# linyicheng1/keypoint_bench

Measured on AMD Instinct MI355X. Metric: image-pairs/sec (extract+NMS+BF-match, 640x480, top_k=1000), higher is better.
Workload: dtype f32

## Files before the change

### include/kpb.h

```cpp
#ifndef KPB_H
#define KPB_H

#include <stddef.h>
#include <stdint.h>

#ifdef __cplusplus
extern "C" {
#endif

#define KPB_VERSION 1

#define KPB_OK 0
#define KPB_E_INVALID (-1)
#define KPB_E_HIP (-2)
#define KPB_E_NOMEM (-3)
#define KPB_E_NEGATIVE (-4)
#define KPB_E_NOT_CONVERGED (-5)
#define KPB_E_WEIGHTS (-6)
#define KPB_E_UNSUPPORTED (-7)

#define KPB_MAX_NMS_DIST 16
#define KPB_MAX_TOPK 8192

typedef struct kpb_ctx kpb_ctx;
// ... 1 lines not shown

typedef struct kpb_detect_params {
    int32_t nms_dist;
    float threshold;
    int32_t border_dist;
    int32_t top_k;
    float min_score;
} kpb_detect_params;

typedef struct kpb_match_params {
    double max_distance;
    int32_t cross_check;
} kpb_match_params;

int kpb_version(void);
const char* kpb_last_error(const kpb_ctx* ctx);

int kpb_ctx_create(int device, void* stream, kpb_ctx** out);
int kpb_ctx_set_stream(kpb_ctx* ctx, void* stream);
void kpb_ctx_destroy(kpb_ctx* ctx);
int kpb_sync(kpb_ctx* ctx);

#define KPB_OPT_COVIS_STORE_BYTES 1
int kpb_ctx_set_option(kpb_ctx* ctx, int option, int64_t value);

int kpb_prof_enable(kpb_ctx* ctx, int on);
int kpb_prof_report(kpb_ctx* ctx, char* buf, size_t cap);

int kpb_fast_nms(kpb_ctx* ctx, const float* score_dev, int batch, int H, int W, int nms_dist,
                 float* out_map_dev);

int kpb_detect(kpb_ctx* ctx, const float* score_dev, int batch, int H, int W,
               const kpb_detect_params* params, float* out_kps_dev, int32_t* out_idx_dev,
               int32_t* out_n_dev, int sync);
int kpb_detect_check(kpb_ctx* ctx);
int kpb_detect_counts(kpb_ctx* ctx, int32_t* out_n_host, int batch);

int kpb_sample(kpb_ctx* ctx, const float* desc_dev, int batch, int C, int Hd, int Wd, int64_t sb,
               int64_t sc, int64_t sh, int64_t sw, const float* pts_dev, int pts_cols, int max_n,
               const int32_t* n_dev, float* out_dev);

int kpb_match(kpb_ctx* ctx, const float* d0_dev, const float* d1_dev, int batch, int C, int max_n,
              int max_m, const int32_t* n_dev, const int32_t* m_dev, const kpb_match_params* params,
              int32_t* out_pairs_dev, double* out_dist_dev, int32_t* out_k_dev);

int kpb_match_counts(kpb_ctx* ctx, int32_t* out_k_host, int batch);
// ... 92 lines not shown
```

### keypoint_bench_amd/_lib.py

```python
import ctypes
import os

_HERE = os.path.dirname(os.path.abspath(__file__))
SO_PATH = os.environ.get("KPB_LIB_PATH") or os.path.join(_HERE, "libkpb.so")

c_int, c_float, c_double, c_void_p, c_int64, c_size_t = (ctypes.c_int, ctypes.c_float, ctypes.c_double,
                                                       ctypes.c_void_p, ctypes.c_int64, ctypes.c_size_t)


class DetectParams(ctypes.Structure):
    _fields_ = [("nms_dist", ctypes.c_int32), ("threshold", c_float), ("border_dist", ctypes.c_int32),
                ("top_k", ctypes.c_int32), ("min_score", c_float)]


class LgParams(ctypes.Structure):
    _fields_ = [("depth_confidence", c_float), ("width_confidence", c_float), ("filter_threshold", c_float),
                ("prune_min_kpts", ctypes.c_int32)]


class LkParams(ctypes.Structure):
    _fields_ = [("distance", ctypes.c_float), ("win_size", ctypes.c_int32), ("levels", ctypes.c_int32), ("iterations", ctypes.c_int32)]


class RansacParams(ctypes.Structure):
# ... 106 lines not shown
    @classmethod
    def get(cls, device):
        import torch
        idx = device.index if isinstance(device, torch.device) else int(device)
        if idx is None:
            idx = torch.cuda.current_device()
        if idx not in cls._instances:
            cls._instances[idx] = cls(idx)
        inst = cls._instances[idx]
        stream = torch.cuda.current_stream(idx).cuda_stream
        if stream != inst.stream:
            inst.check(inst.lib.kpb_ctx_set_stream(inst.handle, c_void_p(stream)))
            inst.stream = stream
        return inst

    def check(self, rc):
        if rc != 0:
            raise KpbError(rc, self.lib.kpb_last_error(self.handle).decode())

    def sync(self):
        self.check(self.lib.kpb_sync(self.handle))

    OPT_COVIS_STORE_BYTES = 1

    def set_option(self, option: int, value: int):
        self.check(self.lib.kpb_ctx_set_option(self.handle, int(option), int(value)))

    def prof_enable(self, on: bool):
        self.check(self.lib.kpb_prof_enable(self.handle, 1 if on else 0))

    def prof_report(self):
        buf = ctypes.create_string_buffer(1 << 16)
        self.check(self.lib.kpb_prof_report(self.handle, buf, len(buf)))
        out = {}
        for line in buf.value.decode().splitlines():
            name, calls, ms = line.split()
            out[name] = (int(calls), float(ms))
        return out


def ptr(t):
    return c_void_p(t.data_ptr()) if t is not None else c_void_p(0)
```

### keypoint_bench_amd/csrc/alike.hip

```cpp
#include "conv_mfma.h"

namespace {

typedef _Float16 h8v __attribute__((ext_vector_type(8)));
typedef _Float16 h2v __attribute__((ext_vector_type(2)));
typedef float f32x4v __attribute__((ext_vector_type(4)));

__device__ __forceinline__ float relu(float v);

__device__ __forceinline__ void split4(const float4 v, uint2& hi, uint2& lo) { cm_split4(v, hi, lo); }

__device__ __forceinline__ void amax_commit(float lane_max, float* slots, int slot, int lane)
{
    const float m = cm_wave_max(lane_max);
    if (lane == 0) slots[slot] = m;
}

__global__ __launch_bounds__(256) void amax_reduce(const float* slots, int n, unsigned* out)
{
    __shared__ float s[4];
    const int b = blockIdx.x, tid = threadIdx.x;
    float m = 0.0f;
    for (int i = tid; i < n; i += 256) {
        const float v = slots[(size_t)b * n + i];
// ... 752 lines not shown

std::vector<float> pack_h16(const float* w, int CIN, const float* ds_w, float scale)
{
    const int OCT = CIN / 8, NK = 9 * OCT + (ds_w ? 1 : 0), KB = (NK + 3) / 4;
    std::vector<uint16_t> hl((size_t)KB * 2 * 64 * 8, 0);
    for (int kb = 0; kb < KB; ++kb)
        for (int l = 0; l < 64; ++l)
            for (int j = 0; j < 8; ++j) {
                const int n = l & 15, g = l >> 4, kidx = 4 * kb + g;
                float v = 0.0f;
                if (kidx < 9 * OCT) { const int tap = kidx / OCT, o = kidx - tap * OCT; v = w[((size_t)n * CIN + 8 * o + j) * 9 + tap]; }
                else if (ds_w && kidx == 9 * OCT) v = ds_w[n * 8 + j];
                v *= scale;
                _Float16 hi = (_Float16)v;
                const _Float16 lo = (_Float16)(v - (float)hi);
                memcpy(&hl[(((size_t)kb * 2 + 0) * 64 + l) * 8 + j], &hi, 2);
                memcpy(&hl[(((size_t)kb * 2 + 1) * 64 + l) * 8 + j], &lo, 2);
            }
    std::vector<float> out(hl.size() / 2);
    memcpy(out.data(), hl.data(), hl.size() * 2);
    return out;
}

constexpr int ESTRIDE = 68;

template <int CIN>
__device__ __forceinline__ void conv1x1_relu_body(const float* __restrict__ in, float* __restrict__ out, const float* __restrict__ w ,
                                                  const float* __restrict__ wsg , float* __restrict__ smap, size_t npix,
                                                  const float* __restrict__ wproj , float* __restrict__ E ,
                                                  const unsigned bx )
{
    const size_t p = (size_t)bx * 256 + threadIdx.x;
    const bool live = p < npix;
    constexpr bool STAGE_IN = CIN <= 32;
    constexpr int XP = CIN + 4;
    constexpr int WREG = STAGE_IN && 64 * XP > 16 * ESTRIDE ? 64 * XP : 16 * ESTRIDE;
    __shared__ __attribute__((aligned(16))) float wlds[4][WREG];
    float* wreg = wlds[threadIdx.x >> 6];
    float acc[16];
#pragma unroll
    for (int j = 0; j < 16; ++j) acc[j] = 0.0f;
    const float* x = in + (live ? p : 0) * CIN;
    if (STAGE_IN) {
        const int ln = threadIdx.x & 63;
        const size_t pw = (size_t)bx * 256 + (threadIdx.x >> 6) * 64;
        float4 ld[CIN / 4];
#pragma unroll
// ... 821 lines not shown
    for (int o = 0; o < co; ++o)
        for (int c = 0; c < ci; ++c) out[(size_t)c * co + o] = w[(size_t)o * ci + c];
}
float l1_rows(const float* w, int co, int per)
{
    float m = 0.0f;
    for (int o = 0; o < co; ++o) {
        double s = 0.0;
        for (int i = 0; i < per; ++i) s += std::fabs((double)w[(size_t)o * per + i]);
        m = std::max(m, (float)(s * (1.0 + 1e-6)));
    }
    return m;
}
float max_abs(const float* b, int n)
{
    float m = 0.0f;
    for (int i = 0; i < n; ++i) m = std::max(m, std::fabs(b[i]));
    return m;
}

constexpr CmForm CM_C16{.ks = 3, .s = 1, .cc = 16, .ntb = 1, .mt = 2, .wn = 2}, CM_C32{.ks = 3, .s = 1, .cc = 32, .ntb = 1, .mt = 4, .wn = 2},
                 CM_C32_1T{.ks = 3, .s = 1, .cc = 32, .ntb = 1}, CM_C16_LAT{.ks = 3, .s = 1, .cc = 16, .wpre = true},
                 CM_C32_LAT{.ks = 3, .s = 1, .cc = 32, .ntb = 1, .wpre = true}, CM_P4_LAT{.ks = 3, .s = 1, .cc = 32, .pool_in = true, .ntb = 1, .pf = 4, .wpre = true};

template <int CIN, int COUT, int POOL, bool RES, int CDS, int RPOOL, bool DSOUT = false, int TW = 32>
void launch_conv(kpb_ctx* ctx, const char* name, hipStream_t st, const ConvArgs& a, int B)
{
    constexpr int G = COUT / 16, TH = (64 / TW) * (4 / G);
    KPB_LAUNCH(ctx, name, (conv3x3_k<CIN, COUT, POOL, RES, CDS, RPOOL, true, DSOUT, TW>), dim3(cdiv(a.W, TW), cdiv(a.H, TH), B), dim3(256), 0, st, a);
}

__global__ __launch_bounds__(256) void maxpool4_nhwc(const float* __restrict__ in, float* __restrict__ out, int Ho, int Wo, int C)
{
    const int C4 = C / 4;
    const size_t i = (size_t)blockIdx.x * 256 + threadIdx.x, b = blockIdx.y;
    if (i >= (size_t)Ho * Wo * C4) return;
    const int c = (int)(i % C4) * 4;
    const size_t pix = i / C4;
    const int y = (int)(pix / Wo), x = (int)(pix - (size_t)y * Wo);
    const float* s = in + ((b * 4 * Ho + 4 * y) * (size_t)(4 * Wo) + 4 * x) * C + c;
    float4 m = *reinterpret_cast<const float4*>(s);
#pragma unroll
    for (int py = 0; py < 4; ++py)
#pragma unroll
        for (int px = 0; px < 4; ++px) {
            if (py == 0 && px == 0) continue;
            const float4 v = *reinterpret_cast<const float4*>(s + ((size_t)py * 4 * Wo + px) * C);
            m.x = fmaxf(m.x, v.x); m.y = fmaxf(m.y, v.y); m.z = fmaxf(m.z, v.z); m.w = fmaxf(m.w, v.w);
        }
    *reinterpret_cast<float4*>(out + ((b * Ho + y) * (size_t)Wo + x) * C + c) = m;
}

int AlikeNet::forward(const float* img_dev, int batch, int H_, int W_, float* score_out_dev, float* desc_out_dev)
{
    if ((H_ % 32) || (W_ % 32))
        return kpb_fail(ctx, KPB_E_INVALID, "kpb_net_forward: ALIKE needs H and W multiples of 32 (got %dx%d)", H_, W_);
    const int H = H_, W = W_;
    const size_t P = (size_t)H * W, B = batch;
    const bool h16 = conv_mfma_use_h16();
    const bool dense = desc_out_dev != nullptr;
    const int nw1 = cdiv(W, B1_TW) * cdiv(H, B1H_TH) * 4, nw2 = cdiv(W / 2, 32) * cdiv(H / 2, 8) * 4;
    const size_t n_2 = B * (P / 4) * 16, n_3 = B * (P / 64) * 32, n_4 = B * (P / 1024) * 64;
    float *p1, *t2, *x2, *t3, *x3, *t4, *x4, *r3, *r4, *t3r3, *t4r4, *p2, *p3, *S2, *S3, *S4, *E3, *E4, *wmax_x1, *wmax_a2;
    unsigned *amax_x1, *amax_a2;
    if (int rc = kpb_carve(ctx, act, [&](Arena& a) {
            auto f32 = [&](size_t n) { return h16 ? nullptr : a.take(n); };
            auto f16 = [&](size_t n) { return h16 ? a.take(n) : nullptr; };
            x1 = a.take(B * P * 8);
            p1 = a.take(B * (P / 4) * 8);
            t2 = f32(n_2); x2 = f32(n_2); a2 = a.take(n_2);
            t3 = f32(n_3); x3 = a.take(n_3); a3 = a.take(B * (P / 64) * 16);
            t4 = f32(n_4); x4 = a.take(n_4); a4 = a.take(B * (P / 1024) * 16);
            r3 = f32(n_3); r4 = f32(n_4);
            t3r3 = f16(2 * n_3);
            t4r4 = f16(2 * n_4);
            p2 = f16(n_3 / 2);
            p3 = h16 && batch >= 16 ? a.take(n_4 / 2) : nullptr;
            S2 = a.take(B * (P / 4)); S3 = a.take(B * (P / 64)); S4 = a.take(B * (P / 1024));
            E3 = dense ? a.take(B * (P / 64) * ESTRIDE) : nullptr;
            E4 = dense ? a.take(B * (P / 1024) * ESTRIDE) : nullptr;
            amax_x1 = h16 ? a.take<unsigned>(B) : nullptr;
            amax_a2 = h16 ? a.take<unsigned>(B) : nullptr;
            wmax_x1 = f16(B * nw1);
            wmax_a2 = f16(B * nw2);
        }))
        return rc;
    this->B = batch; this->H = H; this->W = W;
    hipStream_t st = ctx->stream;

    Block1Args b1{img_dev, x1, p1, k1.w1, k1.b1, k1.w2, k1.b2, H, W};
    ConvArgs c;
    if (h16) {
        Block1HArgs hb{b1, k1.w1pk, k1.w2pk, k1.inv_ws1, k1.inv_ws2, k1.l1_c1, k1.bmax_c1, wmax_x1, 0};
        KPB_LAUNCH(ctx, "alike_block1", alike_block1_h, dim3(cdiv(W, B1_TW), cdiv(H, B1H_TH), batch), dim3(256), 0, st, hb);
        KPB_LAUNCH(ctx, "amax_reduce", amax_reduce, dim3(batch), dim3(256), 0, st, wmax_x1, nw1, amax_x1);
        Block2Args b2{p1, x2, a2, S2, p2, k2.w1pk, k2.w2pk, k2.wapk, k2.b1, k2.bsum, kh.wsc + 16, H / 2, W / 2,
                      k2.inv_ws1, k2.inv_ws2, k2.inv_wsa, k2.l1_c1, k2.bmax_c1, k2.l1_c2, k2.l1_ds, k2.bmax_sum, amax_x1, wmax_a2, 1};
        KPB_LAUNCH(ctx, "alike_block2", alike_block2, dim3(cdiv(W / 2, 32), cdiv(H / 2, 8), batch), dim3(256), 0, st, b2);
        KPB_LAUNCH(ctx, "amax_reduce", amax_reduce, dim3(batch), dim3(256), 0, st, wmax_a2, nw2, amax_a2);
        auto block_h = [&](const Res& r, const float* in, float* tr, float* xo, int cin, int cout, int Hi, int Wi, bool prepooled) {
            ConvM m{.in = in, .out = tr, .wp = r.w1h, .bias = r.b1h, .Hi = prepooled ? Hi / 4 : Hi, .Wi = prepooled ? Wi / 4 : Wi,
                    .H = Hi / 4, .W = Wi / 4, .CIN = cin, .COUT = 2 * cout, .NCH = 1, .relu = 2, .nblk = cout / 32, .istride = cin, .ostride = 2 * cout,
                    .unscale = r.un1, .relu_nt = cout / 32};
            auto launch = [&](const char* prof, const CmForm& f, const ConvM& cm) {
                return launch_conv_mfma_h<CM_C16, CM_C32, CM_C32_1T, CM_C16_LAT, CM_C32_LAT, CM_P4_LAT>(ctx, prof, f, cm, batch); };
            if (batch < 16 && !prepooled) m.nblk = 2 * cout / 32;
            const CmForm f1 = !prepooled ? CM_P4_LAT : batch < 16 ? CM_C16_LAT : cin == 32 ? CM_C32 : CM_C16;
            if (int rc = launch(r.prof1.c_str(), f1, m)) return rc;
            const ConvM c2{.in = tr, .out = xo, .wp = r.w2p, .bias = r.b2p, .res = tr + cout, .Hi = Hi / 4, .Wi = Wi / 4,
                           .H = Hi / 4, .W = Wi / 4, .CIN = cout, .COUT = cout, .NCH = cout / 32, .nblk = batch < 16 ? cout / 32 : 1, .istride = 2 * cout,
                           .ostride = cout, .unscale = r.un2, .rstride = 2 * cout};
            return launch(r.prof2.c_str(), batch < 16 ? CM_C32_LAT : cout == 32 ? CM_C32_1T : CM_C32, c2);
        };
        if (int rc = block_h(blk[3], p2, t3r3, x3, 16, 32, H / 2, W / 2, true)) return rc;
        if (batch >= 16) {
            KPB_LAUNCH(ctx, "maxpool4_x3", maxpool4_nhwc, dim3((unsigned)(((size_t)(H / 32) * (W / 32) * 8 + 255) / 256), batch), dim3(256), 0, st, x3, p3, H / 32, W / 32, 32);
            if (int rc = block_h(blk[4], p3, t4r4, x4, 32, 64, H / 8, W / 8, true)) return rc;
        } else if (int rc = block_h(blk[4], x3, t4r4, x4, 32, 64, H / 8, W / 8, false))
            return rc;
    } else {
        auto conv2 = [&](const Res& r, const float* in, float* out, const float* res, int h, int w, int c) {
            const ConvM m{.in = in, .out = out, .wp = r.w2p, .bias = r.b2p, .res = res, .Hi = h, .Wi = w, .H = h, .W = w,
                          .CIN = c, .COUT = c, .NCH = c / 32, .nblk = 1, .istride = c, .ostride = c};
            return launch_conv_mfma<CmForm{.ks = 3, .s = 1, .cc = 32, .ntb = 1}, CmForm{.ks = 3, .s = 1, .cc = 32}>(
                ctx, r.prof2.c_str(), CmForm{.ks = 3, .s = 1, .cc = 32, .ntb = c / 32}, m, batch);
        };
        KPB_LAUNCH(ctx, "alike_block1", alike_block1, dim3(cdiv(W, B1_TW), cdiv(H, B1_TH), batch), dim3(256), 0, st, b1);
        c = ConvArgs{p1, t2, blk[2].w1, blk[2].b1, nullptr, nullptr, nullptr, nullptr, H / 2, W / 2};
        launch_conv<8, 16, 1, false, 4, 1>(ctx, "conv3x3_b2c1", st, c, batch);
        c = ConvArgs{t2, x2, blk[2].w2, blk[2].b2, p1, blk[2].dsw, blk[2].dsb, nullptr, H / 2, W / 2};
        launch_conv<16, 16, 1, true, 8, 1>(ctx, "conv3x3_b2c2", st, c, batch);
        c = ConvArgs{x2, t3, blk[3].w1, blk[3].b1, nullptr, blk[3].dsw, blk[3].dsb, r3, H / 8, W / 8};
        launch_conv<16, 32, 4, false, 4, 1, true, 16>(ctx, "conv3x3_b3c1", st, c, batch);
        if (int rc = conv2(blk[3], t3, x3, r3, H / 8, W / 8, 32)) return rc;
        c = ConvArgs{x3, t4, blk[4].w1, blk[4].b1, nullptr, blk[4].dsw, blk[4].dsb, r4, H / 32, W / 32};
        launch_conv<32, 64, 4, false, 4, 1, true, 16>(ctx, "conv3x3_b4c1", st, c, batch);
        if (int rc = conv2(blk[4], t4, x4, r4, H / 32, W / 32, 64)) return rc;
        KPB_LAUNCH(ctx, "conv1x1_agg2", conv1x1_relu<16>, dim3((unsigned)((B * P / 4 + 255) / 256)), dim3(256), 0, st, x2, a2, kh.agg[2], kh.wsc + 16, S2, B * P / 4, nullptr, nullptr);
    }
    if (batch < 16) {
        const AggArgs g3{x3, a3, kh.agg[3], kh.wsc + 32, S3, B * P / 64, kh.whT + 32 * 64, E3};
        const AggArgs g4{x4, a4, kh.agg[4], kh.wsc + 48, S4, B * P / 1024, kh.whT + 48 * 64, E4};
        const unsigned nb3 = (unsigned)((B * P / 64 + 255) / 256), nb4 = (unsigned)((B * P / 1024 + 255) / 256);
        KPB_LAUNCH(ctx, "conv1x1_agg34", conv1x1_relu_34, dim3(nb3 + nb4), dim3(256), 0, st, g3, g4, nb3);
    } else {
        KPB_LAUNCH(ctx, "conv1x1_agg3", conv1x1_relu<32>, dim3((unsigned)((B * P / 64 + 255) / 256)), dim3(256), 0, st, x3, a3, kh.agg[3], kh.wsc + 32, S3, B * P / 64, kh.whT + 32 * 64, E3);
        KPB_LAUNCH(ctx, "conv1x1_agg4", conv1x1_relu<64>, dim3((unsigned)((B * P / 1024 + 255) / 256)), dim3(256), 0, st, x4, a4, kh.agg[4], kh.wsc + 48, S4, B * P / 1024, kh.whT + 48 * 64, E4);
    }
    if (dense) {
        HybArgs hy{x1, a2, E3, E4, kh.agg[1], kh.whT, kh.wsc, score_out_dev, desc_out_dev, H, W, amax_x1, amax_a2, 0.f, 1.f, 1.f, nullptr, 1.f};
        const int work4 = cdiv(H, 4) * cdiv(W / 32, SEG_TILES);
        if (h16) {
            hy.l1_agg1 = kh.l1_agg1; hy.inv_ws_h = kh.inv_ws_h; hy.ws_h = 1.0f / hy.inv_ws_h;
            hy.a1h16 = kh.a1h16; hy.inv_wa = kh.inv_wa;
            if (!hp_ring_rows_ok(H, H / 2, HP_A2R) || !hp_ring_rows_ok(H, H / 8, HP_ER) || !hp_ring_rows_ok(H, H / 32, HP_ER))
                return kpb_fail(ctx, KPB_E_UNSUPPORTED, "alike head: the LDS rings cannot hold the source rows of %d row groups at height %d", HP_LA + 1, H);
            const int bands_ = cdiv(W / 32, HP_TILES), groups_ = H / 4;
            const int hp = std::max(2, std::min(30, (int)(((long long)bands_ * groups_ * batch) / 1536)));
            KPB_LAUNCH(ctx, "alike_head_dense", alike_head_f16p, dim3(cdiv(W / 32, HP_TILES) * cdiv(H / 4, hp), batch), dim3(256), 0, st, hy,
                       kh.wh16, hp);
        } else
            KPB_LAUNCH(ctx, "alike_head_dense", alike_head_hyb, dim3(work4, batch), dim3(256), 0, st, hy);
    } else {
// ... 185 lines not shown
```

### keypoint_bench_amd/csrc/api.hip

```cpp
#include "kpb_common.h"

char g_kpb_err[512] = {0};

extern "C" __attribute__((visibility("default"))) int kpb_version(void) { return KPB_VERSION; }

extern "C" __attribute__((visibility("default"))) const char* kpb_last_error(const kpb_ctx* ctx) { return ctx ? ctx->err : g_kpb_err; }

extern "C" __attribute__((visibility("default"))) int kpb_ctx_create(int device, void* stream, kpb_ctx** out)
{
    if (!out) return kpb_fail(nullptr, KPB_E_INVALID, "kpb_ctx_create: null out pointer");
    *out = nullptr;
    int count = 0;
    if (hipGetDeviceCount(&count) != hipSuccess || count == 0)
        return kpb_fail(nullptr, KPB_E_HIP, "kpb_ctx_create: no HIP device visible (this library has no CPU path)");
    if (device < 0 || device >= count)
        return kpb_fail(nullptr, KPB_E_INVALID, "kpb_ctx_create: device %d out of range (0..%d)", device, count - 1);
    hipDeviceProp_t prop;
    KPB_HIP(nullptr, hipGetDeviceProperties(&prop, device));
    if (strncmp(prop.gcnArchName, "gfx950", 6) != 0)
        return kpb_fail(nullptr, KPB_E_HIP, "kpb_ctx_create: device %d is %s; libkpb.so is built for gfx950 only", device,
                        prop.gcnArchName);
    KPB_HIP(nullptr, hipSetDevice(device));
    kpb_ctx* c = new kpb_ctx();
    c->device = device;
// ... 12 lines not shown
    if (ctx->wait_ev) (void)hipEventDestroy(ctx->wait_ev);
    if (ctx->host_det) (void)hipHostFree(ctx->host_det);
    if (ctx->host_match) (void)hipHostFree(ctx->host_match);
    if (ctx->own_stream) (void)hipStreamDestroy(ctx->stream);
    if (ctx->det_state && ctx->det_state_free) ctx->det_state_free(ctx->det_state);
    for (hipEvent_t e : ctx->prof_pool) (void)hipEventDestroy(e);
    delete ctx;
}

extern "C" __attribute__((visibility("default"))) int kpb_ctx_set_stream(kpb_ctx* ctx, void* stream)
{
    if (!ctx) return kpb_fail(nullptr, KPB_E_INVALID, "kpb_ctx_set_stream: null context");
    KPB_HIP(ctx, hipStreamSynchronize(ctx->stream));
    ctx->stream = static_cast<hipStream_t>(stream);
    return KPB_OK;
}

extern "C" __attribute__((visibility("default"))) int kpb_ctx_set_option(kpb_ctx* ctx, int option, int64_t value)
{
    if (!ctx) return kpb_fail(nullptr, KPB_E_INVALID, "kpb_ctx_set_option: null context");
    if (value < 0) return kpb_fail(ctx, KPB_E_INVALID, "kpb_ctx_set_option: negative value");
    switch (option) {
    case KPB_OPT_COVIS_STORE_BYTES: ctx->covis_store_bytes = (size_t)value; return KPB_OK;
    default: return kpb_fail(ctx, KPB_E_INVALID, "kpb_ctx_set_option: unknown option %d", option);
    }
}

extern "C" __attribute__((visibility("default"))) int kpb_sync(kpb_ctx* ctx)
{
    if (!ctx) return kpb_fail(nullptr, KPB_E_INVALID, "kpb_sync: null context");
    KPB_HIP(ctx, hipStreamSynchronize(ctx->stream));
    return KPB_OK;
}

extern "C" __attribute__((visibility("default"))) int kpb_prof_enable(kpb_ctx* ctx, int on)
{
    if (!ctx) return kpb_fail(nullptr, KPB_E_INVALID, "kpb_prof_enable: null context");
    ctx->prof = on != 0;
    return KPB_OK;
}

extern "C" __attribute__((visibility("default"))) int kpb_prof_report(kpb_ctx* ctx, char* buf, size_t cap)
{
    if (!ctx || !buf || cap == 0) return kpb_fail(ctx, KPB_E_INVALID, "kpb_prof_report: bad argument");
    KPB_HIP(ctx, hipStreamSynchronize(ctx->stream));
    std::vector<std::string> names;
// ... 23 lines not shown
```

### keypoint_bench_amd/csrc/conv_mfma.h

```cpp
#pragma once
#include <type_traits>
#include "net.h"

#include <algorithm>
#include <cmath>
#include <cstring>

namespace {

typedef float f32x16 __attribute__((ext_vector_type(16)));

__device__ __forceinline__ float relu(float v) { return fmaxf(v, 0.0f); }

struct ConvM {
    const float* in = nullptr;
    float* out = nullptr;
    const float* wp = nullptr;
    const float* bias = nullptr;
    const float* xf = nullptr;
    const int* active = nullptr;
    const float* res = nullptr;
    int Hi = 0, Wi = 0, H = 0, W = 0, CIN = 0, COUT = 0, NCH = 0, relu = 0, nblk = 0;
    int istride = 0, ostride = 0, ooff = 0;
    float unscale = 1.0f;
    int relu_nt = 0;
    int rstride = 0;
    const float* xw = nullptr;
    float xun = 1.0f;
    const float* gen_w = nullptr; const float* gen_b = nullptr;
    float xb = 0.0f;
    int xco = 0;
    const int* rowcnt = nullptr;
    const float* aux0 = nullptr;
    const float* aux1 = nullptr;
    float* out1 = nullptr;
    float* out2 = nullptr;
    const unsigned* pre_amax = nullptr; float pre_l1 = 0.0f, pre_bmax = 0.0f;
    const float* up_src = nullptr; int up_c = 0;
    int unfold_w = 0;
    int tap_dil = 0;
};

enum { GE_PLAIN = 0, GE_RESIDUAL = 1, GE_ROTARY = 2, GE_SPLIT2 = 3, GE_L2NORM = 4 };

struct CmForm {
    int ks, s, cc;
    bool pool_in, pool_out;
    bool xf;
    int ntb = 2;
    int mt = 1;
    bool xc = false;
    int pf = 2;
    bool wpre = false;
    bool pre = false;
    int wn = 1;
    bool gen = false;
    bool up = false;
    int dil = 1;
    constexpr bool operator==(const CmForm&) const = default;
    constexpr int tile_h() const { return 8 * mt / wn; }
    constexpr int waves() const { return wpre ? 1 : dil > 1 ? 2  : mt * ntb >= 4 ? ((ks == 5 && cc == 32) || pool_in ? 2 : 3) : (mt * ntb == 2 ? (ks == 3 && cc == 16 ? 3 : 4) : 5); }
};

template <CmForm F>
__global__ __launch_bounds__(256) void conv_mfma(ConvM a)
{
    constexpr int KS = F.ks, S = F.s, CC = F.cc, NTB = F.ntb; constexpr bool POOL_IN = F.pool_in, POOL_OUT = F.pool_out, XF = F.xf;
    constexpr int DIL = F.dil;
    static_assert(F == CmForm{.ks = KS, .s = S, .cc = CC, .pool_in = POOL_IN, .pool_out = POOL_OUT, .xf = XF, .ntb = NTB, .dil = DIL},
                  "conv_mfma: the strict-fp32 kernel has no mt, xc, pf, wpre, pre, wn, gen or up");
    constexpr int KC = CC / 2, PITCH = CC + 4, T = KS * KS, PAD = (KS - 1) * DIL / 2;
    constexpr int IH = 7 * S + (KS - 1) * DIL + 1, IW = 15 * S + (KS - 1) * DIL + 1, Q = CC / 4;
    static_assert(IH * IW * PITCH * 4 <= 65536, "conv_mfma: input tile exceeds the static LDS window");
    constexpr int NLD = (IH * IW * Q + 255) / 256;
    __shared__ __attribute__((aligned(16))) float tile[IH * IW * PITCH];
    const int tid = threadIdx.x, lane = tid & 63, wv = tid >> 6, p = lane & 31, h = lane >> 5;
    const int b = blockIdx.z / a.nblk, nb = blockIdx.z - b * a.nblk, nt0 = nb * NTB;
    const int ty0 = blockIdx.y * 8, tx0 = blockIdx.x * 16;
    const int Hc = POOL_IN ? a.Hi / 2 : a.Hi, Wc = POOL_IN ? a.Wi / 2 : a.Wi;
    const int iy0 = ty0 * S - PAD, ix0 = tx0 * S - PAD;
    if (a.active && !a.active[b]) return;
    const float* in = a.in + (size_t)b * a.Hi * a.Wi * a.istride;
    const int orow = 2 * wv + (p >> 4), ocol = p & 15;
    const size_t ntile_stride = (size_t)T * a.NCH * 2 * 32 * KC;

    f32x16 acc[NTB];
#pragma unroll
    for (int n = 0; n < NTB; ++n)
#pragma unroll
        for (int r = 0; r < 16; ++r) acc[n][r] = 0.0f;
    for (int ch = 0; ch < a.NCH; ++ch) {
        __syncthreads();
        {
// ... 145 lines not shown
        return fmaxf(x, __int_as_float(y));
    };
    v = step(v, std::integral_constant<int, 0xB1>{}, std::integral_constant<int, 0xF>{});
    v = step(v, std::integral_constant<int, 0x4E>{}, std::integral_constant<int, 0xF>{});
    v = step(v, std::integral_constant<int, 0x141>{}, std::integral_constant<int, 0xF>{});
    v = step(v, std::integral_constant<int, 0x140>{}, std::integral_constant<int, 0xF>{});
    v = step(v, std::integral_constant<int, 0x142>{}, std::integral_constant<int, 0xA>{});
    v = step(v, std::integral_constant<int, 0x143>{}, std::integral_constant<int, 0xC>{});
    return __int_as_float(__builtin_amdgcn_readlane(__float_as_int(v), 63));
}

__device__ __forceinline__ void cm_up2_taps(int o, int n, int& i0, int& i1, float& l)
{
    const float f = fmaxf(((float)o + 0.5f) * 0.5f - 0.5f, 0.0f);
    i0 = (int)f;
    i1 = i0 + (i0 < n - 1 ? 1 : 0);
    l = f - (float)i0;
}
__device__ __forceinline__ float4 cm_up2_mix(const float4 p00, const float4 p01, const float4 p10, const float4 p11, float ly, float lx)
{
    const float hy = 1.0f - ly, hx = 1.0f - lx;
    return make_float4(hy * (hx * p00.x + lx * p01.x) + ly * (hx * p10.x + lx * p11.x), hy * (hx * p00.y + lx * p01.y) + ly * (hx * p10.y + lx * p11.y),
                       hy * (hx * p00.z + lx * p01.z) + ly * (hx * p10.z + lx * p11.z), hy * (hx * p00.w + lx * p01.w) + ly * (hx * p10.w + lx * p11.w));
}

template <CmForm F>
__global__ __launch_bounds__(256, F.waves()) void conv_mfma_h(ConvM a)
{
    constexpr int KS = F.ks, S = F.s, CC = F.cc, NTB = F.ntb, MT = F.mt, PF = F.pf, WN = F.wn, DIL = F.dil;
    constexpr bool POOL_IN = F.pool_in, POOL_OUT = F.pool_out, XF = F.xf, XC = F.xc, WPRE = F.wpre, PRE = F.pre, GEN = F.gen, UP = F.up;
    static_assert(DIL == 1 || (DIL >= 2 && S == 1 && !WPRE && !PRE && !UP && !XC && !POOL_IN && MT >= 2 && NTB == 1), "conv_mfma_h: the dilated form exists for plain stride-1 layers (R2D2)");
    static_assert(!UP || (S == 1 && !POOL_IN && !PRE && !WPRE && (((F.tile_h() - 1) * S + KS) % 2 == 0) && ((15 * S + KS) % 2 == 0) && KS / 2 % 2 == 0),
                  "conv_mfma_h<UP>: stride-1 layers whose input tile starts on an even row and column");
    static_assert(WN == 1 || (WN == 2 && MT % 2 == 0 && !WPRE), "conv_mfma_h: waves split the n-tiles two ways at most");
    static_assert(PRE == GEN && (!GEN || KS == 3), "conv_mfma_h: the pre-split tile exists as the generated one (a 3 x 3 one-channel layer computed while staging); r05's DMA-landed form was measured, superseded and removed in r06");
    static_assert(!PRE || (CC == 32 && S == 1 && !POOL_IN && !XF && !XC && !WPRE), "conv_mfma_h: the pre-split input form exists for plain stride-1 32-channel slabs");
    constexpr int KC = CC / 2, NKB = CC / 16, T = KS * KS, PAD = (KS - 1) * DIL / 2, TH = F.tile_h();
    constexpr int TAPU = (KS == 3 && !WPRE && !PRE) ? 9 : 1;
    constexpr bool ROW_AHEAD = TAPU == 1 && !WPRE && !PRE;
    constexpr int IH = (TH - 1) * S + (KS - 1) * DIL + 1, IW = 15 * S + (KS - 1) * DIL + 1, Q = CC / 4;
    constexpr int PITCH = 4 * CC + 16, LO = 2 * CC;
    constexpr int ROWP = (IW * PITCH + 255) / 256 * 256;
    constexpr int NLD = (IH * IW * Q + 255) / 256;
    static_assert(IH * ROWP <= 65536, "conv_mfma_h: input tile exceeds the static LDS window");
    __shared__ __attribute__((aligned(256))) unsigned char tile[IH * ROWP];
    const int tid = threadIdx.x, lane = tid & 63, wv = tid >> 6, p = lane & 31, h = lane >> 5;
// ... 364 lines not shown
#pragma unroll
                    for (int j = 0; j < 4; ++j) {
                        const uint2 w = xwq[4 * q + j];
                        xpart = __builtin_amdgcn_fdot2(__builtin_bit_cast(cm_h2, ll[j]), __builtin_bit_cast(cm_h2, w.x), xpart, false);
                        xpart = __builtin_amdgcn_fdot2(__builtin_bit_cast(cm_h2, hh[j]), __builtin_bit_cast(cm_h2, w.y), xpart, false);
                        xpart = __builtin_amdgcn_fdot2(__builtin_bit_cast(cm_h2, hh[j]), __builtin_bit_cast(cm_h2, w.x), xpart, false);
                    }
                }
            }
        }
        }
        if (XC && nb == 0) xacc = fmaf(xpart, cm_unscale_of(e_cur), xacc);
    }
    if (XC && nb == 0) {
        const int gy = ty0 + (tid >> 4), gx = tx0 + (tid & 15);
        if (gy < a.H && gx < a.W) {
            float o = fmaf(xacc, a.xun, a.xb);
            if (a.relu) o = relu(o);
            a.out[(size_t)b * a.H * a.W * a.ostride + a.ooff + ((size_t)gy * a.W + gx) * a.ostride + a.xco] = o;
        }
    }
    const float unscale = a.unscale * cm_unscale_of(e_cur);

#pragma unroll
    for (int m = 0; m < MT; ++m) {
        const int trow = 2 * (wm * MT + m);
#pragma unroll
        for (int n = 0; n < NTB; ++n) {
            const int co = (nt0 + n) * 32 + p;
            const float bias = biasv[n];
            float v[16];
#pragma unroll
            for (int r = 0; r < 16; ++r) {
                v[r] = fmaf(acc[m][n][r], unscale, bias);
                if (a.relu == 1 || (a.relu == 2 && nt0 + n < a.relu_nt)) v[r] = relu(v[r]);
            }
            if (co >= a.COUT) continue;
            if (!POOL_OUT) {
                float* out = a.out + (size_t)b * a.H * a.W * a.ostride + a.ooff;
                const int rs = a.rstride ? a.rstride : a.COUT;
                const float* res = a.res ? a.res + (size_t)b * a.H * a.W * rs : nullptr;
#pragma unroll
                for (int r = 0; r < 16; ++r) {
                    const int i = (r & 3) + 8 * (r >> 2) + 4 * h;
                    const int gy = ty0 + trow + (i >> 4), gx = tx0 + (i & 15);
                    if (gy < a.H && gx < a.W) {
// ... 11 lines not shown
                const int gy = (ty0 + trow) / 2;
#pragma unroll
                for (int cc = 0; cc < 4; ++cc) {
                    const int c = 2 * h + (cc & 1) + 4 * (cc >> 1);
                    const int rA = 2 * (cc & 1) + 4 * (cc >> 1);
                    const int gx = tx0 / 2 + c;
                    if (gy < Ho && gx < Wo)
                        out[((size_t)gy * Wo + gx) * a.ostride + co] = fmaxf(fmaxf(v[rA], v[rA + 1]), fmaxf(v[rA + 8], v[rA + 9]));
                }
            }
        }
    }
}

template <bool H, CmForm... FS>
int cm_launch(kpb_ctx* ctx, const char* tag, const CmForm& f, const ConvM& a, int B)
{
    const bool found = ((f == FS && [&] {
        const dim3 grid(cdiv(a.W, 16), cdiv(a.H, FS.tile_h()), B * a.nblk);
        if constexpr (H) KPB_LAUNCH(ctx, tag, conv_mfma_h<FS>, grid, dim3(256), 0, ctx->stream, a);
        else KPB_LAUNCH(ctx, tag, conv_mfma<FS>, grid, dim3(256), 0, ctx->stream, a);
        return true;
    }()) || ...);
    return found ? KPB_OK : kpb_fail(ctx, KPB_E_INVALID, "%s: no instance for %s: ks=%d s=%d cc=%d pool_in=%d pool_out=%d xf=%d ntb=%d mt=%d xc=%d pf=%d wpre=%d pre=%d wn=%d gen=%d up=%d dil=%d",
        H ? "conv_mfma_h" : "conv_mfma", tag, f.ks, f.s, f.cc, f.pool_in, f.pool_out, f.xf, f.ntb, f.mt, f.xc, f.pf, f.wpre, f.pre, f.wn, f.gen, f.up, f.dil);
}
template <CmForm... FS> int launch_conv_mfma_h(kpb_ctx* ctx, const char* tag, const CmForm& f, const ConvM& a, int B) { return cm_launch<true, FS...>(ctx, tag, f, a, B); }
template <CmForm... FS> int launch_conv_mfma(kpb_ctx* ctx, const char* tag, const CmForm& f, const ConvM& a, int B) { return cm_launch<false, FS...>(ctx, tag, f, a, B); }

template <int NTB, int MT = 2, int EPI = GE_PLAIN, bool UNFOLD = false, int TAPK = 0>
__global__ __launch_bounds__(256, MT == 1 ? (EPI == GE_ROTARY || TAPK ? 3 : 4) : 2) void gemm_h(ConvM a)
{
    constexpr int CC = 32, KC = 16, NKB = 2, Q = CC / 4, PITCH = 4 * CC + 16, LO = 2 * CC, WROWS = 32 * MT, ROWS = 4 * WROWS, WBUF = WROWS * PITCH,
                  NLD = WROWS * Q / 64;
    __shared__ __attribute__((aligned(256))) unsigned char tile[2 * 4 * WBUF];
    const int tid = threadIdx.x, lane = tid & 63, wv = tid >> 6, p = lane & 31, h = lane >> 5;
    const int b = blockIdx.z / a.nblk, nb = blockIdx.z - b * a.nblk, nt0 = nb * NTB;
    if (a.active && !a.active[b]) return;
    const int nrows_all = a.H * a.W, r0 = blockIdx.x * ROWS + WROWS * wv;
    const int nrows = a.rowcnt ? min(nrows_all, a.rowcnt[b]) : nrows_all;
    if (r0 >= nrows) return;
    if ((EPI == GE_RESIDUAL || EPI == GE_ROTARY) && blockIdx.x * ROWS + ROWS > nrows_all) return;
    const float* in = a.in + (size_t)b * nrows_all * a.istride;
    const uint4* wq = reinterpret_cast<const uint4*>(a.wp);
    const size_t ntile_stride = (size_t)a.NCH * NKB * 4 * 32;
    unsigned char* wt = tile + wv * WBUF;
    float biasv[NTB];
#pragma unroll
// ... 309 lines not shown
```

### keypoint_bench_amd/csrc/kpb_common.h

```cpp
#pragma once
#include <hip/hip_runtime.h>

#include <cstdarg>
#include <cstdint>
#include <cstdio>
#include <cstdlib>
#include <cstring>
#include <set>
#include <string>
#include <vector>
#include <type_traits>

#include "../../include/kpb.h"
#include <chrono>

__device__ __forceinline__ void kpb_halves32(float v, float& lo, float& hi)
{
    const auto r = __builtin_amdgcn_permlane32_swap(__float_as_uint(v), __float_as_uint(v), false, false);
    lo = __uint_as_float(r[0]);
    hi = __uint_as_float(r[1]);
}
struct kpb_tile3 { int x, y, z; };
__device__ __forceinline__ kpb_tile3 kpb_xcd_tile(int enable)
{
// ... 92 lines not shown
    std::vector<hipEvent_t> prof_pool;
    std::set<std::string> prof_names;
    hipStream_t stream = nullptr;
    bool own_stream = false;
    char err[512] = {0};
    kpb_buf ws_nms_state;
    kpb_buf ws_nms_map;
    kpb_buf ws_nms_list;
    kpb_buf ws_cand;
    kpb_buf ws_match;
    kpb_buf ws_misc;
    kpb_buf ws_sel;
    int* host_det = nullptr;
    int host_det_cap = 0;
    hipEvent_t wait_ev = nullptr;
    int* host_match = nullptr;
    int host_match_cap = 0, host_match_n = 0;
    void* det_state = nullptr;
    void (*det_state_free)(void*) = nullptr;
    int det_pending = 0;
    int det_counts_valid = 0, match_counts_valid = 0;
    unsigned lds_attr_done = 0;
    size_t covis_store_bytes = (size_t)4 << 30;
};
enum { KPB_ATTR_NMS = 1u, KPB_ATTR_HOMOGRAPHY = 2u, KPB_ATTR_ESSENTIAL = 4u, KPB_ATTR_FUNDAMENTAL = 8u };

extern char g_kpb_err[512];

inline int kpb_fail(kpb_ctx* ctx, int code, const char* fmt, ...)
{
    char* dst = ctx ? ctx->err : g_kpb_err;
    va_list ap;
    va_start(ap, fmt);
    vsnprintf(dst, 512, fmt, ap);
    va_end(ap);
    return code;
}

#define KPB_HIP(ctx, call)                                                                             \
    do {                                                                                               \
        hipError_t e_ = (call);                                                                        \
        if (e_ != hipSuccess)                                                                          \
            return kpb_fail(ctx, KPB_E_HIP, "%s failed: %s (%s:%d)", #call, hipGetErrorString(e_),     \
                            __FILE__, __LINE__);                                                       \
    } while (0)

// ... 90 lines not shown
```

Measured before the change: 15810.

## Fuse ALIKE coarse-block aggregation and max-pool into conv2 MFMA epilogue

Adds a tail epilogue to the half-precision MFMA conv kernel for ALIKE blocks 3 and 4. The residual output tile stays in LDS, where it is max-pooled for the next block and run through the 1x1 aggregation, score and projection heads, so x3/x4 are never written to global memory and the separate maxpool and aggregation launches go away. It is gated by a new context option that defaults on, for batch >= 16 with h16. The cost is more LDS and register pressure in the conv kernel, and work per block that is serialized across waves.

```diff
diff --git a/include/kpb.h b/include/kpb.h
--- a/include/kpb.h
+++ b/include/kpb.h
@@ -47,6 +47,7 @@
 int kpb_sync(kpb_ctx* ctx);
 
 #define KPB_OPT_COVIS_STORE_BYTES 1
+#define KPB_OPT_ALIKE_COARSE_FUSED 2
 int kpb_ctx_set_option(kpb_ctx* ctx, int option, int64_t value);
 
 int kpb_prof_enable(kpb_ctx* ctx, int on);
diff --git a/keypoint_bench_amd/_lib.py b/keypoint_bench_amd/_lib.py
--- a/keypoint_bench_amd/_lib.py
+++ b/keypoint_bench_amd/_lib.py
@@ -152,6 +152,7 @@
         self.check(self.lib.kpb_sync(self.handle))
 
     OPT_COVIS_STORE_BYTES = 1
+    OPT_ALIKE_COARSE_FUSED = 2
 
     def set_option(self, option: int, value: int):
         self.check(self.lib.kpb_ctx_set_option(self.handle, int(option), int(value)))
diff --git a/keypoint_bench_amd/csrc/alike.hip b/keypoint_bench_amd/csrc/alike.hip
--- a/keypoint_bench_amd/csrc/alike.hip
+++ b/keypoint_bench_amd/csrc/alike.hip
@@ -798,7 +798,7 @@
     return out;
 }
 
-constexpr int ESTRIDE = 68;
+constexpr int ESTRIDE = CM_ESTRIDE;
 
 template <int CIN>
 __device__ __forceinline__ void conv1x1_relu_body(const float* __restrict__ in, float* __restrict__ out, const float* __restrict__ w ,
@@ -1666,6 +1666,7 @@
 constexpr CmForm CM_C16{.ks = 3, .s = 1, .cc = 16, .ntb = 1, .mt = 2, .wn = 2}, CM_C32{.ks = 3, .s = 1, .cc = 32, .ntb = 1, .mt = 4, .wn = 2},
                  CM_C32_1T{.ks = 3, .s = 1, .cc = 32, .ntb = 1}, CM_C16_LAT{.ks = 3, .s = 1, .cc = 16, .wpre = true},
                  CM_C32_LAT{.ks = 3, .s = 1, .cc = 32, .ntb = 1, .wpre = true}, CM_P4_LAT{.ks = 3, .s = 1, .cc = 32, .pool_in = true, .ntb = 1, .pf = 4, .wpre = true};
+constexpr CmForm CM_B3C2_TAIL{.ks = 3, .s = 1, .cc = 32, .ntb = 1, .tail = 2}, CM_B4C2_TAIL{.ks = 3, .s = 1, .cc = 32, .ntb = 1, .mt = 4, .wn = 2, .tail = 1};
 
 template <int CIN, int COUT, int POOL, bool RES, int CDS, int RPOOL, bool DSOUT = false, int TW = 32>
 void launch_conv(kpb_ctx* ctx, const char* name, hipStream_t st, const ConvArgs& a, int B)
@@ -1703,6 +1704,7 @@
     const size_t P = (size_t)H * W, B = batch;
     const bool h16 = conv_mfma_use_h16();
     const bool dense = desc_out_dev != nullptr;
+    const bool fused = h16 && batch >= 16 && ctx->alike_coarse_fused;
     const int nw1 = cdiv(W, B1_TW) * cdiv(H, B1H_TH) * 4, nw2 = cdiv(W / 2, 32) * cdiv(H / 2, 8) * 4;
     const size_t n_2 = B * (P / 4) * 16, n_3 = B * (P / 64) * 32, n_4 = B * (P / 1024) * 64;
     float *p1, *t2, *x2, *t3, *x3, *t4, *x4, *r3, *r4, *t3r3, *t4r4, *p2, *p3, *S2, *S3, *S4, *E3, *E4, *wmax_x1, *wmax_a2;
@@ -1713,8 +1715,8 @@
             x1 = a.take(B * P * 8);
             p1 = a.take(B * (P / 4) * 8);
             t2 = f32(n_2); x2 = f32(n_2); a2 = a.take(n_2);
-            t3 = f32(n_3); x3 = a.take(n_3); a3 = a.take(B * (P / 64) * 16);
-            t4 = f32(n_4); x4 = a.take(n_4); a4 = a.take(B * (P / 1024) * 16);
+            t3 = f32(n_3); x3 = fused ? nullptr : a.take(n_3); a3 = a.take(B * (P / 64) * 16);
+            t4 = f32(n_4); x4 = fused ? nullptr : a.take(n_4); a4 = a.take(B * (P / 1024) * 16);
             r3 = f32(n_3); r4 = f32(n_4);
             t3r3 = f16(2 * n_3);
             t4r4 = f16(2 * n_4);
@@ -1742,22 +1744,32 @@
                       k2.inv_ws1, k2.inv_ws2, k2.inv_wsa, k2.l1_c1, k2.bmax_c1, k2.l1_c2, k2.l1_ds, k2.bmax_sum, amax_x1, wmax_a2, 1};
         KPB_LAUNCH(ctx, "alike_block2", alike_block2, dim3(cdiv(W / 2, 32), cdiv(H / 2, 8), batch), dim3(256), 0, st, b2);
         KPB_LAUNCH(ctx, "amax_reduce", amax_reduce, dim3(batch), dim3(256), 0, st, wmax_a2, nw2, amax_a2);
-        auto block_h = [&](const Res& r, const float* in, float* tr, float* xo, int cin, int cout, int Hi, int Wi, bool prepooled) {
+        auto block_h = [&](const Res& r, const float* in, float* tr, float* xo, int cin, int cout, int Hi, int Wi, bool prepooled, int gi = 0, float* ao = nullptr,
+                           float* So = nullptr, float* Eo = nullptr, float* pool = nullptr) {
             ConvM m{.in = in, .out = tr, .wp = r.w1h, .bias = r.b1h, .Hi = prepooled ? Hi / 4 : Hi, .Wi = prepooled ? Wi / 4 : Wi,
                     .H = Hi / 4, .W = Wi / 4, .CIN = cin, .COUT = 2 * cout, .NCH = 1, .relu = 2, .nblk = cout / 32, .istride = cin, .ostride = 2 * cout,
                     .unscale = r.un1, .relu_nt = cout / 32};
             auto launch = [&](const char* prof, const CmForm& f, const ConvM& cm) {
-                return launch_conv_mfma_h<CM_C16, CM_C32, CM_C32_1T, CM_C16_LAT, CM_C32_LAT, CM_P4_LAT>(ctx, prof, f, cm, batch); };
+                return launch_conv_mfma_h<CM_C16, CM_C32, CM_C32_1T, CM_C16_LAT, CM_C32_LAT, CM_P4_LAT, CM_B3C2_TAIL, CM_B4C2_TAIL>(ctx, prof, f, cm, batch); };
             if (batch < 16 && !prepooled) m.nblk = 2 * cout / 32;
             const CmForm f1 = !prepooled ? CM_P4_LAT : batch < 16 ? CM_C16_LAT : cin == 32 ? CM_C32 : CM_C16;
             if (int rc = launch(r.prof1.c_str(), f1, m)) return rc;
-            const ConvM c2{.in = tr, .out = xo, .wp = r.w2p, .bias = r.b2p, .res = tr + cout, .Hi = Hi / 4, .Wi = Wi / 4,
-                           .H = Hi / 4, .W = Wi / 4, .CIN = cout, .COUT = cout, .NCH = cout / 32, .nblk = batch < 16 ? cout / 32 : 1, .istride = 2 * cout,
-                           .ostride = cout, .unscale = r.un2, .rstride = 2 * cout};
+            ConvM c2{.in = tr, .out = xo, .wp = r.w2p, .bias = r.b2p, .res = tr + cout, .Hi = Hi / 4, .Wi = Wi / 4,
+                     .H = Hi / 4, .W = Wi / 4, .CIN = cout, .COUT = cout, .NCH = cout / 32, .nblk = batch < 16 ? cout / 32 : 1, .istride = 2 * cout,
+                     .ostride = cout, .unscale = r.un2, .rstride = 2 * cout};
+            if (ao) {
+                c2.tl_w = kh.agg[gi]; c2.tl_wsg = kh.wsc + 16 * (gi - 1); c2.tl_wproj = kh.whT + 16 * (gi - 1) * 64;
+                c2.tl_agg = ao; c2.tl_smap = So; c2.tl_E = Eo; c2.tl_pool = pool;
+                return launch(r.prof2.c_str(), pool ? CM_B3C2_TAIL : CM_B4C2_TAIL, c2);
+            }
             return launch(r.prof2.c_str(), batch < 16 ? CM_C32_LAT : cout == 32 ? CM_C32_1T : CM_C32, c2);
         };
-        if (int rc = block_h(blk[3], p2, t3r3, x3, 16, 32, H / 2, W / 2, true)) return rc;
-        if (batch >= 16) {
+        if (fused) {
+            if (int rc = block_h(blk[3], p2, t3r3, nullptr, 16, 32, H / 2, W / 2, true, 3, a3, S3, E3, p3)) return rc;
+            if (int rc = block_h(blk[4], p3, t4r4, nullptr, 32, 64, H / 8, W / 8, true, 4, a4, S4, E4)) return rc;
+        } else if (int rc = block_h(blk[3], p2, t3r3, x3, 16, 32, H / 2, W / 2, true))
+            return rc;
+        else if (batch >= 16) {
             KPB_LAUNCH(ctx, "maxpool4_x3", maxpool4_nhwc, dim3((unsigned)(((size_t)(H / 32) * (W / 32) * 8 + 255) / 256), batch), dim3(256), 0, st, x3, p3, H / 32, W / 32, 32);
             if (int rc = block_h(blk[4], p3, t4r4, x4, 32, 64, H / 8, W / 8, true)) return rc;
         } else if (int rc = block_h(blk[4], x3, t4r4, x4, 32, 64, H / 8, W / 8, false))
@@ -1782,7 +1794,9 @@
         if (int rc = conv2(blk[4], t4, x4, r4, H / 32, W / 32, 64)) return rc;
         KPB_LAUNCH(ctx, "conv1x1_agg2", conv1x1_relu<16>, dim3((unsigned)((B * P / 4 + 255) / 256)), dim3(256), 0, st, x2, a2, kh.agg[2], kh.wsc + 16, S2, B * P / 4, nullptr, nullptr);
     }
-    if (batch < 16) {
+    if (fused)
+        ;
+    else if (batch < 16) {
         const AggArgs g3{x3, a3, kh.agg[3], kh.wsc + 32, S3, B * P / 64, kh.whT + 32 * 64, E3};
         const AggArgs g4{x4, a4, kh.agg[4], kh.wsc + 48, S4, B * P / 1024, kh.whT + 48 * 64, E4};
         const unsigned nb3 = (unsigned)((B * P / 64 + 255) / 256), nb4 = (unsigned)((B * P / 1024 + 255) / 256);
diff --git a/keypoint_bench_amd/csrc/api.hip b/keypoint_bench_amd/csrc/api.hip
--- a/keypoint_bench_amd/csrc/api.hip
+++ b/keypoint_bench_amd/csrc/api.hip
@@ -58,6 +58,10 @@
     if (value < 0) return kpb_fail(ctx, KPB_E_INVALID, "kpb_ctx_set_option: negative value");
     switch (option) {
     case KPB_OPT_COVIS_STORE_BYTES: ctx->covis_store_bytes = (size_t)value; return KPB_OK;
+    case KPB_OPT_ALIKE_COARSE_FUSED:
+        if (value > 1) return kpb_fail(ctx, KPB_E_INVALID, "kpb_ctx_set_option: KPB_OPT_ALIKE_COARSE_FUSED takes 0 or 1 (got %lld)", (long long)value);
+        ctx->alike_coarse_fused = (int)value;
+        return KPB_OK;
     default: return kpb_fail(ctx, KPB_E_INVALID, "kpb_ctx_set_option: unknown option %d", option);
     }
 }
diff --git a/keypoint_bench_amd/csrc/conv_mfma.h b/keypoint_bench_amd/csrc/conv_mfma.h
--- a/keypoint_bench_amd/csrc/conv_mfma.h
+++ b/keypoint_bench_amd/csrc/conv_mfma.h
@@ -39,7 +39,10 @@
     const float* up_src = nullptr; int up_c = 0;
     int unfold_w = 0;
     int tap_dil = 0;
+    const float* tl_w = nullptr; const float* tl_wsg = nullptr; const float* tl_wproj = nullptr;
+    float* tl_agg = nullptr; float* tl_smap = nullptr; float* tl_E = nullptr; float* tl_pool = nullptr;
 };
+constexpr int CM_ESTRIDE = 68;
 
 enum { GE_PLAIN = 0, GE_RESIDUAL = 1, GE_ROTARY = 2, GE_SPLIT2 = 3, GE_L2NORM = 4 };
 
@@ -57,9 +60,10 @@
     bool gen = false;
     bool up = false;
     int dil = 1;
+    int tail = 0;
     constexpr bool operator==(const CmForm&) const = default;
     constexpr int tile_h() const { return 8 * mt / wn; }
-    constexpr int waves() const { return wpre ? 1 : dil > 1 ? 2  : mt * ntb >= 4 ? ((ks == 5 && cc == 32) || pool_in ? 2 : 3) : (mt * ntb == 2 ? (ks == 3 && cc == 16 ? 3 : 4) : 5); }
+    constexpr int waves() const { return wpre ? 1 : tail && mt == 4 ? 2 : dil > 1 ? 2  : mt * ntb >= 4 ? ((ks == 5 && cc == 32) || pool_in ? 2 : 3) : (mt * ntb == 2 ? (ks == 3 && cc == 16 ? 3 : 4) : 5); }
 };
 
 template <CmForm F>
@@ -68,7 +72,7 @@
     constexpr int KS = F.ks, S = F.s, CC = F.cc, NTB = F.ntb; constexpr bool POOL_IN = F.pool_in, POOL_OUT = F.pool_out, XF = F.xf;
     constexpr int DIL = F.dil;
     static_assert(F == CmForm{.ks = KS, .s = S, .cc = CC, .pool_in = POOL_IN, .pool_out = POOL_OUT, .xf = XF, .ntb = NTB, .dil = DIL},
-                  "conv_mfma: the strict-fp32 kernel has no mt, xc, pf, wpre, pre, wn, gen or up");
+                  "conv_mfma: the strict-fp32 kernel has no mt, xc, pf, wpre, pre, wn, gen, up or tail");
     constexpr int KC = CC / 2, PITCH = CC + 4, T = KS * KS, PAD = (KS - 1) * DIL / 2;
     constexpr int IH = 7 * S + (KS - 1) * DIL + 1, IW = 15 * S + (KS - 1) * DIL + 1, Q = CC / 4;
     static_assert(IH * IW * PITCH * 4 <= 65536, "conv_mfma: input tile exceeds the static LDS window");
@@ -260,6 +264,68 @@
     const float hy = 1.0f - ly, hx = 1.0f - lx;
     return make_float4(hy * (hx * p00.x + lx * p01.x) + ly * (hx * p10.x + lx * p11.x), hy * (hx * p00.y + lx * p01.y) + ly * (hx * p10.y + lx * p11.y),
                        hy * (hx * p00.z + lx * p01.z) + ly * (hx * p10.z + lx * p11.z), hy * (hx * p00.w + lx * p01.w) + ly * (hx * p10.w + lx * p11.w));
+}
+
+template <int CT>
+__device__ __forceinline__ void cm_tail_agg(const float* x, float* strip, const float* w_ , const float* wsg_ ,
+                                            const float* wproj_ , float* __restrict__ out, float* __restrict__ smap, float* __restrict__ E,
+                                            const size_t (&row_pix)[4], const int (&ncol)[4], int lane, int half)
+{
+    typedef const __attribute__((address_space(4))) float* cfp;
+    const cfp w = (cfp)w_, wsg = (cfp)wsg_, wproj = (cfp)wproj_;
+    float acc[16];
+#pragma unroll
+    for (int j = 0; j < 16; ++j) acc[j] = 0.0f;
+#pragma unroll 2
+    for (int c4 = 0; c4 < CT / 4; ++c4) {
+        const float4 v4 = *reinterpret_cast<const float4*>(x + c4 * 4);
+        const float v[4] = {v4.x, v4.y, v4.z, v4.w};
+#pragma unroll
+        for (int c = 0; c < 4; ++c)
+#pragma unroll
+            for (int j = 0; j < 16; ++j) acc[j] = fmaf(v[c], w[(c4 * 4 + c) * 16 + j], acc[j]);
+    }
+    float sg = 0.0f;
+#pragma unroll
+    for (int j = 0; j < 16; ++j) { acc[j] = relu(acc[j]); sg = fmaf(acc[j], wsg[j], sg); }
+    const int g_own = lane >> 4, col = lane & 15;
+    size_t pix = 0; bool live = false;
+#pragma unroll
+    for (int g = 0; g < 4; ++g)
+        if (g == g_own) { pix = row_pix[g] + col; live = col < ncol[g]; }
+    if (live && half == 0) {
+        float* o = out + pix * 16;
+#pragma unroll
+        for (int q = 0; q < 4; ++q)
+            *reinterpret_cast<float4*>(o + 4 * q) = make_float4(acc[4 * q], acc[4 * q + 1], acc[4 * q + 2], acc[4 * q + 3]);
+        smap[pix] = sg;
+    }
+    if (!E) return;
+#pragma unroll
+    for (int rnd = 0; rnd < 2; ++rnd) {
+        const int q0 = 8 * half + 4 * rnd;
+        float4 r[4];
+#pragma unroll
+        for (int k = 0; k < 4; ++k) {
+            r[k] = make_float4(0.f, 0.f, 0.f, 0.f);
+#pragma unroll
+            for (int c = 0; c < 16; ++c) {
+                const cfp wr = wproj + c * 64 + 4 * (q0 + k);
+                r[k].x = fmaf(acc[c], wr[0], r[k].x); r[k].y = fmaf(acc[c], wr[1], r[k].y);
+                r[k].z = fmaf(acc[c], wr[2], r[k].z); r[k].w = fmaf(acc[c], wr[3], r[k].w);
+            }
+        }
+#pragma unroll
+        for (int g = 0; g < 4; ++g) {
+            if (g_own == g) {
+#pragma unroll
+                for (int k = 0; k < 4; ++k) *reinterpret_cast<float4*>(strip + col * 16 + 4 * k) = r[k];
+            }
+            if ((lane >> 2) < ncol[g])
+                *reinterpret_cast<float4*>(E + (row_pix[g] + (lane >> 2)) * CM_ESTRIDE + 4 * (q0 + (lane & 3))) = *reinterpret_cast<const float4*>(strip + 4 * lane);
+        }
+    }
+    if (live && half == 1) *reinterpret_cast<float4*>(E + pix * CM_ESTRIDE + 64) = make_float4(sg, 0.f, 0.f, 0.f);
 }
 
 template <CmForm F>
@@ -670,6 +736,71 @@
     }
     const float unscale = a.unscale * cm_unscale_of(e_cur);
 
+    if constexpr (F.tail != 0) {
+        static_assert(S == 1 && NTB == 1 && DIL == 1 && !POOL_OUT && !XC && !WPRE && !PRE && !UP && TH % 8 == 0, "conv_mfma_h<tail>: ALIKE's conv2 forms");
+        constexpr int CT = 32 * WN, XP = CT + 4;
+        constexpr int NPASS = TH / 8;
+        static_assert((128 * XP + 4 * 256) * 4 <= IH * ROWP, "conv_mfma_h<tail>: a pass and the four waves' staging strips live in the input tile's LDS");
+        static_assert(F.tail == 1 || (NPASS == 1 && CT == 32), "conv_mfma_h<tail>: the pooling wave takes a 16 x 8 tile of 32 channels");
+        float* xt = reinterpret_cast<float*>(tile);
+        static_assert(MT == 1 || MT == 4, "conv_mfma_h<tail>: a wave's M tiles lie in ONE pass (rows 2 wv .. or 8 wm ..)");
+        const int rs = a.rstride ? a.rstride : a.COUT, co = nt0 * 32 + p;
+        const float* res = a.res + (size_t)b * a.H * a.W * rs + co;
+#pragma unroll
+        for (int pass = 0; pass < NPASS; ++pass) {
+            __syncthreads();
+            if (2 * wm * MT / 8 == pass) {
+#pragma unroll
+                for (int m = 0; m < MT; ++m) {
+                    const int lrow = 2 * (wm * MT + m) - 8 * pass;
+                    float rv[16];
+#pragma unroll
+                    for (int r = 0; r < 16; ++r) {
+                        const int i = (r & 3) + 8 * (r >> 2) + 4 * h;
+                        const int gy = min(ty0 + 8 * pass + lrow + (i >> 4), a.H - 1), gx = min(tx0 + (i & 15), a.W - 1);
+                        rv[r] = res[(gy * a.W + gx) * rs];
+                    }
+#pragma unroll
+                    for (int r = 0; r < 16; ++r) {
+                        const int i = (r & 3) + 8 * (r >> 2) + 4 * h;
+                        float o = fmaf(acc[m][0][r], unscale, biasv[0]);
+                        if (a.relu == 1 || (a.relu == 2 && nt0 < a.relu_nt)) o = relu(o);
+                        xt[((lrow + (i >> 4)) * 16 + (i & 15)) * XP + co] = relu(o + rv[r]);
+                    }
+                    __builtin_amdgcn_sched_barrier(0);
+                }
+            }
+            __syncthreads();
+            if (F.tail == 2 && wv == 2) {
+                const int pp = lane >> 3, q = lane & 7, py = pp >> 2, px = pp & 3;
+                const int Ho = a.H / 4, Wo = a.W / 4, oy = ty0 / 4 + py, ox = tx0 / 4 + px;
+                const float* s = xt + ((4 * py) * 16 + 4 * px) * XP + 4 * q;
+                float4 mx = *reinterpret_cast<const float4*>(s);
+#pragma unroll
+                for (int dy = 0; dy < 4; ++dy)
+#pragma unroll
+                    for (int dx = 0; dx < 4; ++dx) {
+                        if (dy == 0 && dx == 0) continue;
+                        const float4 v = *reinterpret_cast<const float4*>(s + (dy * 16 + dx) * XP);
+                        mx.x = fmaxf(mx.x, v.x); mx.y = fmaxf(mx.y, v.y); mx.z = fmaxf(mx.z, v.z); mx.w = fmaxf(mx.w, v.w);
+                    }
+                if (oy < Ho && ox < Wo) *reinterpret_cast<float4*>(a.tl_pool + (((size_t)b * Ho + oy) * Wo + ox) * CT + 4 * q) = mx;
+            }
+            if (wv < 2 || a.tl_E) {
+                const int wvs = __builtin_amdgcn_readfirstlane(wv), ps = wvs & 1;
+                size_t row_pix[4]; int ncol[4];
+#pragma unroll
+                for (int g = 0; g < 4; ++g) {
+                    const int gy = ty0 + 8 * pass + 4 * ps + g;
+                    row_pix[g] = ((size_t)b * a.H + gy) * a.W + tx0;
+                    ncol[g] = gy < a.H ? min(16, a.W - tx0) : 0;
+                }
+                cm_tail_agg<CT>(xt + (ps * 64 + lane) * XP, xt + 128 * XP + wvs * 256, a.tl_w, a.tl_wsg, a.tl_wproj, a.tl_agg, a.tl_smap, a.tl_E, row_pix, ncol, lane, wvs >> 1);
+            }
+        }
+        return;
+    }
+
 #pragma unroll
     for (int m = 0; m < MT; ++m) {
         const int trow = 2 * (wm * MT + m);
@@ -727,8 +858,8 @@
         else KPB_LAUNCH(ctx, tag, conv_mfma<FS>, grid, dim3(256), 0, ctx->stream, a);
         return true;
     }()) || ...);
-    return found ? KPB_OK : kpb_fail(ctx, KPB_E_INVALID, "%s: no instance for %s: ks=%d s=%d cc=%d pool_in=%d pool_out=%d xf=%d ntb=%d mt=%d xc=%d pf=%d wpre=%d pre=%d wn=%d gen=%d up=%d dil=%d",
-        H ? "conv_mfma_h" : "conv_mfma", tag, f.ks, f.s, f.cc, f.pool_in, f.pool_out, f.xf, f.ntb, f.mt, f.xc, f.pf, f.wpre, f.pre, f.wn, f.gen, f.up, f.dil);
+    return found ? KPB_OK : kpb_fail(ctx, KPB_E_INVALID, "%s: no instance for %s: ks=%d s=%d cc=%d pool_in=%d pool_out=%d xf=%d ntb=%d mt=%d xc=%d pf=%d wpre=%d pre=%d wn=%d gen=%d up=%d dil=%d tail=%d",
+        H ? "conv_mfma_h" : "conv_mfma", tag, f.ks, f.s, f.cc, f.pool_in, f.pool_out, f.xf, f.ntb, f.mt, f.xc, f.pf, f.wpre, f.pre, f.wn, f.gen, f.up, f.dil, f.tail);
 }
 template <CmForm... FS> int launch_conv_mfma_h(kpb_ctx* ctx, const char* tag, const CmForm& f, const ConvM& a, int B) { return cm_launch<true, FS...>(ctx, tag, f, a, B); }
 template <CmForm... FS> int launch_conv_mfma(kpb_ctx* ctx, const char* tag, const CmForm& f, const ConvM& a, int B) { return cm_launch<false, FS...>(ctx, tag, f, a, B); }
diff --git a/keypoint_bench_amd/csrc/kpb_common.h b/keypoint_bench_amd/csrc/kpb_common.h
--- a/keypoint_bench_amd/csrc/kpb_common.h
+++ b/keypoint_bench_amd/csrc/kpb_common.h
@@ -138,6 +138,7 @@
     int det_counts_valid = 0, match_counts_valid = 0;
     unsigned lds_attr_done = 0;
     size_t covis_store_bytes = (size_t)4 << 30;
+    int alike_coarse_fused = 1;
 };
 enum { KPB_ATTR_NMS = 1u, KPB_ATTR_HOMOGRAPHY = 2u, KPB_ATTR_ESSENTIAL = 4u, KPB_ATTR_FUNDAMENTAL = 8u };
 
```

After: 16010, median of 6. +1.3%, better.
